# kumar-shridhar/PyTorch-BayesianCNN

Hardware: AMD Instinct MI355X
Metric: MC-forward samples/sec, BayesianAlexNet CIFAR-10 bs=512 num_ens=10 (higher is better)
Workload: dtype f32; 1 GPU; BayesianAlexNet 3x32x32 -> 10, layer_type=bbb, softplus, bs=512, num_ens=10, forward only; global_batch=512, num_ens_total=10, parallelism=single, launch=hipGraph replay, 2 lane(s) x 4 steps per launch

## Files before the change

### pytorch-bayesiancnn_amd/csrc/pconv_args.h

```cpp
#pragma once
#include <stdint.h>

struct PConvArgs {
    const float* x;
    const float* w;
    const float* w2;
    const float* bias;
    const float* bias2;
    float* y;
    float* y_mu;
    float* y_var;
    const float* eps_ext;
    int64_t x_ds, w_ds, b_ds, y_ds;
    int32_t B, Cin, H, W, Cout, kh, kw, sh, sw, ph, pw, dh, dw, Ho, Wo;
    int32_t K, Kp, khkw, act, sample;
    int32_t Mtiles, nbt, Ntiles, G, per_xcd;
    uint32_t k0, k1, call0, stream_id;
    int32_t wtap;
    uint32_t x_inv;
    const uint32_t* call_dev;
    int32_t unit_div, unit_off, x_mod, b_off;
    int32_t ksplit;
    int32_t* tickets;
    float* part;
    int32_t px_run;
    int64_t x_ps, y_ps;
    int32_t pool;
    int32_t x_div, x_off;
    int32_t y_f32;
    int32_t vh0, vh1, vw0, vw1;
    int32_t y_c8;
    int32_t up_h, up_w, tstep_h, tstep_w;
};
```

### pytorch-bayesiancnn_amd/csrc/pconv_body.cuh

```cuda
#pragma once
#include <hip/hip_runtime.h>
#include <stdint.h>

#include "bbb_common.cuh"
#include "pconv_args.h"

namespace pconv {

typedef float f32x16 __attribute__((ext_vector_type(16)));
typedef float f32x4 __attribute__((ext_vector_type(4)));

constexpr int kThreads = 256;
constexpr int BN = 64;
constexpr int BK = 32;
constexpr int LDW = BN + 1;
constexpr int KCH = 256;
constexpr int TPC = KCH / BK;

constexpr int kPlain = 0, kSplit = 1, kSeq = 2, kPool = 3;

__device__ __forceinline__ float agpr_read(float a) {
    float v;
    asm volatile("v_accvgpr_read_b32 %0, %1" : "=v"(v) : "a"(a));
    return v;
}
__device__ __forceinline__ void agpr_write(float& a, float v) { asm volatile("v_accvgpr_write_b32 %0, %1" : "=a"(a) : "v"(v)); }
template <int BM, bool LRT, bool ILV, int MODE = kPlain, bool TR = false>
__device__ __forceinline__ void pconv_item(const PConvArgs& p, const int64_t item, const int ks = 0) {
    constexpr bool SPLIT = MODE == kSplit;
    constexpr bool SEQ = MODE == kSeq;
    constexpr bool POOL = MODE == kPool;
    static_assert(!POOL || !LRT || BM == 64, "the pooled LRT form: 64-image tiles (one accumulator pair per wave)");
    static_assert(!TR || (MODE == kPlain && !LRT), "the transposed item: plain BBB form only");
    constexpr int LDX = BM + 4;
    constexpr int NT = (BM >= 128) ? 2 : 1;
    constexpr int MT = (BM == 256) ? 2 : 1;
    constexpr int WSETS = LRT ? 2 : 1;
    constexpr int XL = BM / 4;
    constexpr int XRPP = kThreads / XL;
    constexpr int XPASS = BK / XRPP;

    __shared__ __attribute__((aligned(16))) float Xs[1][BK * LDX];
    __shared__ float Ws[1][WSETS][BK * LDW];
    __shared__ int32_t kt_w[2][KCH];
    __shared__ int32_t kt_x[2][KCH];
    __shared__ float sbias[POOL ? BN : 1];
    __shared__ float sbias2[(POOL && LRT) ? BN : 1];

    int g, j;
    if (p.x_ds == 0 || (p.x_div > 1 && p.x_off == 0 && p.G % (p.x_div * p.Ntiles) == 0)) {
        const int gs = p.x_div > 1 ? p.x_div * p.Ntiles : p.G;
        const int64_t per_step = (int64_t)p.Mtiles * gs;
        const int step = (int)(item / per_step);
        const int64_t r = item - (int64_t)step * per_step;
        j = (int)(r / gs);
        g = step * gs + (int)(r - (int64_t)j * gs);
    } else {
        g = (int)(item / p.Mtiles);
        j = (int)(item - (int64_t)g * p.Mtiles);
    }
    const int e = g / p.Ntiles;
    const int ue = p.unit_off + e;
    const int ew = p.unit_div > 1 ? ue / p.unit_div : e;
    const int ex = p.x_div > 1 ? (e + p.x_off) / p.x_div : (p.x_mod > 0 ? ue % p.x_mod : e);
    const int n0 = (g - e * p.Ntiles) * BN;
    const int pix = j / p.nbt;
    const int b0 = (j - pix * p.nbt) * BM;
    const int Wq = POOL ? p.Wo / 2 : p.Wo;
    const int oh0 = pix / Wq, ow0 = pix - oh0 * Wq;
    int ihb, iwb, r_lo, q_lo, nq, nrq, Keff, ntiles;
    float inv_nrq, inv_nq;
    const float inv_cin = 1.0f / (float)p.Cin;
    auto tr_axis = [](int base, int d, int up, int step, int k, int n, int& lo, int& cnt) {
        lo = 0; cnt = 0;
        int first = -1;
        for (int r = 0; r < step && r < k; ++r)
            if ((base + r * d) % up == 0) { first = r; break; }
        if (first < 0) return;
        const int t0 = base + first * d, sd = step * d;
        const int r0 = first + (t0 < 0 ? (-t0 + sd - 1) / sd : 0) * step;
        const int lim = (n - 1) * up - base;
        if (lim < 0) return;
        int r1 = lim / d;
        r1 = r1 < k - 1 ? r1 : k - 1;
        if (r1 < r0) return;
        lo = r0; cnt = (r1 - r0) / step + 1;
    };
    auto set_pixel = [&](int oh, int ow) {
        if constexpr (POOL) {
            oh = __builtin_amdgcn_readfirstlane(oh);
            ow = __builtin_amdgcn_readfirstlane(ow);
        }
        if constexpr (TR) {
            ihb = oh - p.ph;
            iwb = ow - p.pw;
            int nr;
            tr_axis(ihb, p.dh, p.up_h, p.tstep_h, p.kh, p.H, r_lo, nr);
            tr_axis(iwb, p.dw, p.up_w, p.tstep_w, p.kw, p.W, q_lo, nq);
            nrq = nr * nq;
            Keff = p.Cin * nrq;
            ntiles = (Keff + BK - 1) / BK;
            inv_nrq = nrq > 0 ? 1.0f / (float)nrq : 0.0f;
            inv_nq = nq > 0 ? 1.0f / (float)nq : 0.0f;
            return;
        }
        ihb = oh * p.sh - p.ph;
        iwb = ow * p.sw - p.pw;
        r_lo = ihb < 0 ? (-ihb + p.dh - 1) / p.dh : 0;
        q_lo = iwb < 0 ? (-iwb + p.dw - 1) / p.dw : 0;
        int r_hi = (p.H - 1 - ihb) >= 0 ? (p.H - 1 - ihb) / p.dh + 1 : 0;
        int q_hi = (p.W - 1 - iwb) >= 0 ? (p.W - 1 - iwb) / p.dw + 1 : 0;
        r_hi = r_hi < p.kh ? r_hi : p.kh;
        q_hi = q_hi < p.kw ? q_hi : p.kw;
        const int nr = r_hi > r_lo ? r_hi - r_lo : 0;
        nq = q_hi > q_lo ? q_hi - q_lo : 0;
        nrq = nr * nq;
        Keff = p.Cin * nrq;
        ntiles = (Keff + BK - 1) / BK;
        inv_nrq = nrq > 0 ? 1.0f / (float)nrq : 0.0f;
        inv_nq = nq > 0 ? 1.0f / (float)nq : 0.0f;
    };
    set_pixel(POOL ? 2 * oh0 : oh0, POOL ? 2 * ow0 : ow0);

    const int tid = threadIdx.x;
    const int lane = tid & 63;
    const int wave = __builtin_amdgcn_readfirstlane(tid >> 6);
    const int wn = (BM >= 128) ? 0 : (wave >> 1) * 32;
    const int wm = (BM >= 128) ? wave * 32 * MT : (wave & 1) * 32;

    constexpr uint32_t kOOB = 0xFFFFFFF0u;
    constexpr uint32_t kWInv = 0x7FFFFFF0u;
    const uint32_t kXInv = p.x_inv;
    const int64_t w_elems = (int64_t)p.Cout * p.Kp;
    const int64_t x_elems = (int64_t)p.Cin * p.H * p.W * p.B;
    const __amdgpu_buffer_rsrc_t xrs = __builtin_amdgcn_make_buffer_rsrc(
        const_cast<float*>(p.x + (int64_t)ex * p.x_ds), 0, (int)(x_elems * 4), 0x00020000);
    const __amdgpu_buffer_rsrc_t wrs = __builtin_amdgcn_make_buffer_rsrc(
        const_cast<float*>(p.w + (int64_t)ew * p.w_ds), 0, (int)(w_elems * 4), 0x00020000);
    const __amdgpu_buffer_rsrc_t w2rs = __builtin_amdgcn_make_buffer_rsrc(
        const_cast<float*>(LRT ? p.w2 + (int64_t)ew * p.w_ds : p.w), 0, (int)(w_elems * 4), 0x00020000);

    const int wkl = tid & 31, wnl = tid >> 5;
    const int xb4 = (tid % XL) * 4, xkr = tid / XL;
    const uint32_t xcol = (uint32_t)(b0 + xb4) * 4u;
    uint32_t wrow[8];
#pragma unroll
    for (int ps = 0; ps < 8; ++ps) wrow[ps] = (uint32_t)(n0 + wnl + ps * 8) * (uint32_t)p.Kp * 4u;

    float wregA[WSETS][8];
    f32x4 xregA[XPASS];
// ... 4 lines not shown
        if (k < Keff) {
            int ci, rq;
            if (p.wtap) {
                rq = (int)((float)k * inv_cin);
                ci = k - rq * p.Cin;
                if (ci < 0) { --rq; ci += p.Cin; } else if (ci >= p.Cin) { ++rq; ci -= p.Cin; }
            } else {
                ci = (int)((float)k * inv_nrq);
                rq = k - ci * nrq;
                if (rq < 0) { --ci; rq += nrq; } else if (rq >= nrq) { ++ci; rq -= nrq; }
            }
            int rr = (int)((float)rq * inv_nq);
            int qq = rq - rr * nq;
            if (qq < 0) { --rr; qq += nq; } else if (qq >= nq) { ++rr; qq -= nq; }
            if constexpr (TR) {
                const int r = r_lo + rr * p.tstep_h, q = q_lo + qq * p.tstep_w;
                wo = (uint32_t)(ci * p.khkw + r * p.kw + q) * 4u;
                xo = (uint32_t)((ci * p.H + (ihb + r * p.dh) / p.up_h) * p.W + (iwb + q * p.dw) / p.up_w) * (uint32_t)p.B * 4u;
            } else {
                const int r = r_lo + rr, q = q_lo + qq;
                wo = (p.wtap ? (uint32_t)((r * p.kw + q) * p.Cin + ci) : (uint32_t)(ci * p.khkw + r * p.kw + q)) * 4u;
                xo = (uint32_t)((ci * p.H + ihb + r * p.dh) * p.W + iwb + q * p.dw) * (uint32_t)p.B * 4u;
            }
        }
        kt_w[chunk & 1][tid] = (int32_t)wo;
        kt_x[chunk & 1][tid] = (int32_t)xo;
    };

    constexpr int NLOADS = 8 + XPASS;
    uint32_t loff[NLOADS];
    auto load_addr = [&](int tile) {
        const int buf = (tile / TPC) & 1;
        const int kb = (tile % TPC) * BK;
        const uint32_t wob = (uint32_t)kt_w[buf][kb + wkl];
#pragma unroll
        for (int ps = 0; ps < 8; ++ps) loff[ps] = wrow[ps] + wob;
#pragma unroll
        for (int ps = 0; ps < XPASS; ++ps) loff[8 + ps] = (uint32_t)kt_x[buf][kb + xkr + ps * XRPP] + xcol;
    };
    auto load_one = [&](int i, float (&wreg)[WSETS][8], f32x4 (&xreg)[XPASS]) {
        if (i < XPASS) {
            xreg[i] = __builtin_bit_cast(f32x4, __builtin_amdgcn_raw_buffer_load_b128(xrs, loff[8 + i], 0, 0));
        } else {
            const int ps = i - XPASS;
            wreg[0][ps] = __builtin_bit_cast(float, __builtin_amdgcn_raw_buffer_load_b32(wrs, loff[ps], 0, 0));
            if (LRT) wreg[WSETS - 1][ps] = __builtin_bit_cast(float, __builtin_amdgcn_raw_buffer_load_b32(w2rs, loff[ps], 0, 0));
        }
    };
    auto load_tile = [&](int tile, float (&wreg)[WSETS][8], f32x4 (&xreg)[XPASS]) {
        load_addr(tile);
#pragma unroll
        for (int i = 0; i < NLOADS; ++i) load_one(i, wreg, xreg);
    };

    auto store_tile = [&](int, float (&wreg)[WSETS][8], f32x4 (&xreg)[XPASS]) {
        constexpr int buf = 0;
#pragma unroll
        for (int s = 0; s < WSETS; ++s)
#pragma unroll
            for (int ps = 0; ps < 8; ++ps) Ws[buf][s][wkl * LDW + wnl + ps * 8] = wreg[s][ps];
#pragma unroll
        for (int ps = 0; ps < XPASS; ++ps)
            *reinterpret_cast<f32x4*>(&Xs[buf][(xkr + ps * XRPP) * LDX + xb4]) = xreg[ps];
    };

    f32x16 acc[NT][MT];
    f32x16 accv[NT][MT];
    float tot[(SEQ || POOL) ? NT : 1][(SEQ || POOL) ? MT : 1][16];
    float totv[(SEQ && LRT) ? NT : 1][(SEQ && LRT) ? MT : 1][16];
#pragma unroll
    for (int t = 0; t < NT; ++t)
#pragma unroll
        for (int u = 0; u < MT; ++u)
#pragma unroll
            for (int r = 0; r < 16; ++r) {
                acc[t][u][r] = 0.0f; accv[t][u][r] = 0.0f;
                if constexpr (SEQ) { agpr_write(tot[t][u][r], 0.0f); if constexpr (LRT) agpr_write(totv[t][u][r], 0.0f); }
                if constexpr (POOL) agpr_write(tot[t][u][r], -__builtin_inff());
            }

    const int lrow = lane & 31, lk = lane >> 5;

    constexpr int PD = (BM >= 128) ? 2 : 4;
    auto mma_tile = [&](bool more) {
        float ra[PD + 1][NT], ra2[PD + 1][NT], rb[PD + 1][MT];
        auto fetch = [&](int kk, int slot) {
            const int krow = kk * 2 + lk;
#pragma unroll
            for (int mt = 0; mt < MT; ++mt) rb[slot][mt] = Xs[0][krow * LDX + wm + mt * 32 + lrow];
#pragma unroll
            for (int nt = 0; nt < NT; ++nt) {
                ra[slot][nt] = Ws[0][0][krow * LDW + wn + nt * 32 + lrow];
                if (LRT) ra2[slot][nt] = Ws[0][WSETS - 1][krow * LDW + wn + nt * 32 + lrow];
            }
        };
#pragma unroll
        for (int i = 0; i < PD; ++i) fetch(i, i);
#pragma unroll
        for (int kk = 0; kk < BK / 2; ++kk) {
            if (ILV && kk < NLOADS) {
                if (more) load_one(kk, wregA, xregA);
                __builtin_amdgcn_sched_barrier(0);
            }
            if (kk + PD < BK / 2) fetch(kk + PD, (kk + PD) % (PD + 1));
            const int s = kk % (PD + 1);
#pragma unroll
            for (int nt = 0; nt < NT; ++nt) {
#pragma unroll
                for (int mt = 0; mt < MT; ++mt)
                    acc[nt][mt] = __builtin_amdgcn_mfma_f32_32x32x2f32(ra[s][nt], rb[s][mt], acc[nt][mt], 0, 0, 0);
                if (LRT) {
#pragma unroll
                    for (int mt = 0; mt < MT; ++mt)
                        accv[nt][mt] = __builtin_amdgcn_mfma_f32_32x32x2f32(ra2[s][nt], rb[s][mt] * rb[s][mt], accv[nt][mt], 0, 0, 0);
                }
            }
            if (!ILV) __builtin_amdgcn_sched_barrier(0);
        }
    };

    if constexpr (POOL) {
        const __amdgpu_buffer_rsrc_t brs0 = __builtin_amdgcn_make_buffer_rsrc(
            const_cast<float*>(p.bias ? p.bias + (int64_t)ew * p.b_ds : p.w), 0, p.bias ? p.Cout * 4 : 0, 0x00020000);
        if (tid < BN) sbias[tid] = __builtin_bit_cast(float, __builtin_amdgcn_raw_buffer_load_b32(brs0, (uint32_t)(n0 + tid) * 4u, 0, 0));
        if constexpr (LRT) {
            const __amdgpu_buffer_rsrc_t brs2 = __builtin_amdgcn_make_buffer_rsrc(
                const_cast<float*>(p.bias2 ? p.bias2 + (int64_t)ew * p.b_ds : p.w), 0, p.bias2 ? p.Cout * 4 : 0, 0x00020000);
            if (tid < BN) sbias2[tid] = __builtin_bit_cast(float, __builtin_amdgcn_raw_buffer_load_b32(brs2, (uint32_t)(n0 + tid) * 4u, 0, 0));
        }
        __syncthreads();
    }
#pragma clang loop unroll(disable)
    for (int wp = 0; wp < (POOL ? 4 : 1); ++wp) {
    if (POOL && wp > 0) set_pixel(2 * oh0 + (wp >> 1), 2 * ow0 + (wp & 1));
    int t0 = 0, t1 = ntiles;
    if constexpr (SPLIT) {
        t0 = (int)((int64_t)ks * ntiles / p.ksplit);
        t1 = (int)((int64_t)(ks + 1) * ntiles / p.ksplit);
    }
    if (t1 > t0) {
        const int c0 = t0 / TPC;
        fill_chunk(c0);
        __syncthreads();
        load_tile(t0, wregA, xregA);
        if ((c0 + 1) * KCH < Keff) fill_chunk(c0 + 1);
        store_tile(0, wregA, xregA);
        __syncthreads();
        const int nranges = SEQ ? p.ksplit : 1;
        int t = t0;
#pragma clang loop unroll(disable)
        for (int sr = 0; sr < nranges; ++sr) {
            const int tr1 = SEQ ? (int)((int64_t)(sr + 1) * ntiles / p.ksplit) : t1;
#pragma clang loop unroll(disable)
            for (; t < tr1; ++t) {
                const bool more = (t + 1) < t1;
                if (more) {
                    if (ILV) load_addr(t + 1);
                    else     load_tile(t + 1, wregA, xregA);
                }
                if ((t % TPC) == 1 && t / TPC >= c0 + 1 && (t / TPC + 1) * KCH < Keff) fill_chunk(t / TPC + 1);
                mma_tile(more);
                __syncthreads();
                if (more) store_tile(0, wregA, xregA);
                __syncthreads();
            }
            if constexpr (SEQ) {
                if (sr + 1 < nranges) {
#pragma unroll
                    for (int nt = 0; nt < NT; ++nt)
#pragma unroll
                        for (int mt = 0; mt < MT; ++mt)
#pragma unroll
                            for (int r = 0; r < 16; ++r) {
                                agpr_write(tot[nt][mt][r], agpr_read(tot[nt][mt][r]) + acc[nt][mt][r]);
                                acc[nt][mt][r] = 0.0f;
                                if constexpr (LRT) {
                                    agpr_write(totv[nt][mt][r], agpr_read(totv[nt][mt][r]) + accv[nt][mt][r]);
                                    accv[nt][mt][r] = 0.0f;
                                }
                            }
                }
            }
        }
        if constexpr (SEQ) {
#pragma unroll
            for (int nt = 0; nt < NT; ++nt)
#pragma unroll
                for (int mt = 0; mt < MT; ++mt)
#pragma unroll
                    for (int r = 0; r < 16; ++r) {
                        acc[nt][mt][r] = agpr_read(tot[nt][mt][r]) + acc[nt][mt][r];
                        if constexpr (LRT) accv[nt][mt][r] = agpr_read(totv[nt][mt][r]) + accv[nt][mt][r];
                    }
        }
    }
    if constexpr (POOL && !LRT) {
#pragma unroll
        for (int nt = 0; nt < NT; ++nt)
#pragma unroll
            for (int r = 0; r < 16; ++r) {
                const float bn = sbias[wn + nt * 32 + (r & 3) + 8 * (r >> 2) + 4 * lk];
#pragma unroll
                for (int mt = 0; mt < MT; ++mt) {
                    const float v = bbb::apply_act(acc[nt][mt][r] + bn, p.act);
                    agpr_write(tot[nt][mt][r], fmaxf(agpr_read(tot[nt][mt][r]), v));
                    acc[nt][mt][r] = 0.0f;
                }
            }
    }
    if constexpr (POOL && LRT) {
        const int pixc = (2 * oh0 + (wp >> 1)) * p.Wo + 2 * ow0 + (wp & 1);
        const int HoWoC = p.Ho * p.Wo;
#pragma unroll
        for (int mt = 0; mt < MT; ++mt) {
            const int b = b0 + wm + mt * 32 + lrow;
            const int bglob = b + p.b_off + (p.unit_div > 1 ? (ue % p.unit_div) * p.B : 0);
#pragma unroll
            for (int nt = 0; nt < NT; ++nt)
#pragma unroll
                for (int r = 0; r < 16; ++r) {
                    const int nl = wn + nt * 32 + (r & 3) + 8 * (r >> 2) + 4 * lk;
                    const int n = n0 + nl;
                    float v = acc[nt][mt][r] + sbias[nl];
                    const float var = 1e-16f + (accv[nt][mt][r] + sbias2[nl]);
                    if (p.sample) {
                        float z;
                        if (p.eps_ext) {
                            const bool in = (b < p.B) & (n < p.Cout);
                            z = in ? p.eps_ext[(int64_t)e * ((int64_t)p.Cout * HoWoC * p.B) + ((int64_t)n * HoWoC + pixc) * p.B + b] : 0.0f;
                        } else {
                            const uint64_t idx = (uint64_t)(((int64_t)bglob * p.Cout + n) * HoWoC + pixc);
                            float z4[4];
                            bbb::normal4(idx >> 2, p.stream_id, p.call0 + (p.call_dev ? *p.call_dev : 0u) + (uint32_t)ew, p.k0, p.k1, z4);
                            const int c = (int)(idx & 3);
                            z = c == 0 ? z4[0] : c == 1 ? z4[1] : c == 2 ? z4[2] : z4[3];
                        }
                        v = v + __builtin_amdgcn_sqrtf(var) * z;
                    }
                    v = bbb::apply_act(v, p.act);
                    agpr_write(tot[nt][mt][r], fmaxf(agpr_read(tot[nt][mt][r]), v));
                    acc[nt][mt][r] = 0.0f;
                    accv[nt][mt][r] = 0.0f;
                    __builtin_amdgcn_sched_barrier(0);
                }
// ... 197 lines not shown
```

### pytorch-bayesiancnn_amd/csrc/pconv_dgrad.hip

```cpp
#include <hip/hip_runtime.h>
#include <stdint.h>

#include "../../include/bbb_hip.h"
#include "bbb_common.cuh"
#include "pconv_args.h"
#include "pconv_body.cuh"

namespace {

using namespace pconv;

template <int BM, bool ILV>
__global__ __launch_bounds__(kThreads) void pconv_dgrad_kernel(const PConvArgs p) {
    const int bid = blockIdx.x;
    const int xcd = bid & 7;
    const int64_t item = (int64_t)xcd * p.per_xcd + (bid >> 3);
    const int64_t item_end = (int64_t)(xcd + 1) * p.per_xcd;
    if (item >= item_end || item >= (int64_t)p.G * p.Mtiles) return;
    pconv_item<BM, false, ILV, kPlain, true>(p, item);
}

int gcd(int a, int b) {
    while (b != 0) { const int t = a % b; a = b; b = t; }
    return a;
}

}

extern "C" int bbb_conv2d_chwn_dgrad(const bbb_conv_desc_t* d, const float* g_pre, const float* w_flipped, float* dx, int up_h,
                                     int up_w, int out_h, int out_w, void* stream) {
    if (d == nullptr) return BBB_EINVAL;
    if (d->batch <= 0 || d->cin <= 0 || d->h <= 0 || d->w <= 0 || d->cout <= 0 || d->kh <= 0 || d->kw <= 0 || d->pad_h < 0 ||
        d->pad_w < 0 || d->dil_h <= 0 || d->dil_w <= 0 || d->draws <= 0 || up_h <= 0 || up_w <= 0 || out_h <= 0 || out_w <= 0)
        return BBB_EINVAL;
    if (d->stride_h != 1 || d->stride_w != 1) return BBB_EINVAL;
    if (up_h == 1 && up_w == 1) return BBB_EINVAL;
    if (d->act != 0 || d->pool != 0 || d->w_tap_major != 0 || d->w_row_pitch != 0 || d->unit_div != 0 || d->unit_off != 0 ||
        d->x_unit_mod != 0 || d->x_unit_div != 0 || d->x_unit_off != 0 || d->b_offset != 0)
        return BBB_EINVAL;
    if (d->x_draw_stride < 0 || d->w_draw_stride < 0) return BBB_EINVAL;
    if (d->batch % 4 != 0) return BBB_ESHAPE;
    const int fph = d->dil_h * (d->kh - 1) - d->pad_h, fpw = d->dil_w * (d->kw - 1) - d->pad_w;
    if (fph < 0 || fpw < 0) return BBB_ESHAPE;
    const int64_t nh = (int64_t)out_h + 2 * fph - (int64_t)d->dil_h * (d->kh - 1) - 1;
    const int64_t nw = (int64_t)out_w + 2 * fpw - (int64_t)d->dil_w * (d->kw - 1) - 1;
    if (nh < 0 || nw < 0 || nh / up_h + 1 != d->h || nw / up_w + 1 != d->w) return BBB_ESHAPE;
    const int64_t g_bytes = (int64_t)d->cin * d->h * d->w * d->batch * 4, dx_bytes = (int64_t)d->cout * out_h * out_w * d->batch * 4;
    if ((int64_t)d->cin * d->h * d->w > 0x7fffffffLL || (int64_t)d->cin * d->kh * d->kw > 0x7fffffffLL) return BBB_ESHAPE;
    if (g_bytes > 0xFFFE0000LL || dx_bytes > 0xFFFE0000LL || ((int64_t)d->cout + 64) * d->cin * d->kh * d->kw * 4 > 0x3FFFFFFFLL ||
        (int64_t)d->batch * 4 > 0x0FFFFFFFLL)
        return BBB_ESHAPE;
    PConvArgs a = {};
    a.x_inv = (0xFFFFFFF0u - ((uint32_t)d->batch + 512u) * 4u) & ~15u;
    if (g_bytes > (int64_t)a.x_inv) return BBB_ESHAPE;
    if (g_pre == nullptr || w_flipped == nullptr || dx == nullptr) return BBB_EINVAL;
    if ((((uintptr_t)g_pre | (uintptr_t)dx) & 15u) != 0 || (((uintptr_t)w_flipped) & 3u) != 0) return BBB_EALIGN;
    a.x = g_pre; a.w = w_flipped; a.y = dx;
    a.B = d->batch; a.Cin = d->cin; a.H = d->h; a.W = d->w; a.Cout = d->cout; a.kh = d->kh; a.kw = d->kw;
    a.sh = 1; a.sw = 1; a.ph = d->pad_h; a.pw = d->pad_w; a.dh = d->dil_h; a.dw = d->dil_w;
    a.Ho = out_h; a.Wo = out_w; a.K = d->cin * d->kh * d->kw; a.Kp = a.K; a.khkw = d->kh * d->kw;
    a.x_ds = d->x_draw_stride; a.w_ds = d->w_draw_stride;
    a.y_ds = (int64_t)d->cout * out_h * out_w * d->batch;
    a.up_h = up_h; a.up_w = up_w;
    a.tstep_h = up_h / gcd(up_h, d->dil_h); a.tstep_w = up_w / gcd(up_w, d->dil_w);
    a.Ntiles = (a.Cout + BN - 1) / BN;
    a.G = a.Ntiles * d->draws;
    const int64_t pixels = (int64_t)out_h * out_w;
    const int64_t nb128 = pixels * ((a.B + 127) / 128) * a.G;
    int bm = nb128 < 768 ? 64 : 128;
    if (bm == 128 && (a.B + 127) / 128 * 128 * 4 >= a.B * 5 && (a.B + 63) / 64 * 64 < (a.B + 127) / 128 * 128) bm = 64;
    a.nbt = (a.B + bm - 1) / bm;
    const int64_t mt = pixels * a.nbt;
    if (mt > 0x7fffffffLL) return BBB_ESHAPE;
    a.Mtiles = (int)mt;
    const int64_t items = (int64_t)a.G * mt;
    const int64_t per = (items + 7) / 8;
    if (8 * per > 0x7fffffffLL) return BBB_ESHAPE;
    a.per_xcd = (int32_t)per;
    const bool ilv = items <= 12000;
    const dim3 grid((unsigned)(8 * per)), block(kThreads);
    hipStream_t st = (hipStream_t)stream;
    if (bm == 128) {
        if (ilv) hipLaunchKernelGGL((pconv_dgrad_kernel<128, true>), grid, block, 0, st, a);
        else     hipLaunchKernelGGL((pconv_dgrad_kernel<128, false>), grid, block, 0, st, a);
    } else {
        if (ilv) hipLaunchKernelGGL((pconv_dgrad_kernel<64, true>), grid, block, 0, st, a);
        else     hipLaunchKernelGGL((pconv_dgrad_kernel<64, false>), grid, block, 0, st, a);
    }
    return (int)hipGetLastError();
}
```

### pytorch-bayesiancnn_amd/csrc/pconv_gemm.hip

```cpp
#include <hip/hip_runtime.h>
#include <stdlib.h>
#include <stdint.h>

#include "../../include/bbb_hip.h"
#include "bbb_common.cuh"
#include "pconv_args.h"
#include "pconv_body.cuh"
#include "pconv_bf16x3.cuh"

namespace {

using namespace pconv;

template <int BM, bool LRT, bool ILV, bool SEQ = false>
__global__ __launch_bounds__(kThreads) void pconv_gemm_kernel(const PConvArgs p) {
    const int bid = blockIdx.x;
    const int xcd = bid & 7;
    const int64_t item = (int64_t)xcd * p.per_xcd + (bid >> 3);
    const int64_t item_end = (int64_t)(xcd + 1) * p.per_xcd;
    if (item >= item_end || item >= (int64_t)p.G * p.Mtiles) return;
    pconv_item<BM, LRT, ILV, SEQ ? kSeq : kPlain>(p, item);
}

template <bool ILV>
__global__ __launch_bounds__(kThreads) __attribute__((amdgpu_waves_per_eu(4, 4))) void pconv_gemm_pool_kernel(const PConvArgs p) {
    const int bid = blockIdx.x;
    const int xcd = bid & 7;
    const int64_t item = (int64_t)xcd * p.per_xcd + (bid >> 3);
    const int64_t item_end = (int64_t)(xcd + 1) * p.per_xcd;
    if (item >= item_end || item >= (int64_t)p.G * p.Mtiles) return;
    pconv_item<128, false, ILV, kPool>(p, item);
}

__global__ __launch_bounds__(kThreads) void pconv_gemm_pool_lrt_kernel(const PConvArgs p) {
    const int bid = blockIdx.x;
    const int xcd = bid & 7;
    const int64_t item = (int64_t)xcd * p.per_xcd + (bid >> 3);
    const int64_t item_end = (int64_t)(xcd + 1) * p.per_xcd;
    if (item >= item_end || item >= (int64_t)p.G * p.Mtiles) return;
    pconv_item<64, true, false, kPool>(p, item);
}

template <int BM, bool LRT, bool ILV>
__global__ __launch_bounds__(kThreads) void pconv_gemm_splitk_kernel(const PConvArgs p) {
    const int bid = blockIdx.x;
    const int xcd = bid & 7;
    const int64_t blk = (int64_t)xcd * p.per_xcd + (bid >> 3);
    const int64_t blk_end = (int64_t)(xcd + 1) * p.per_xcd;
    if (blk >= blk_end || blk >= (int64_t)p.G * p.Mtiles * p.ksplit) return;
    const int64_t item = blk / p.ksplit;
    pconv_item<BM, LRT, ILV, kSplit>(p, item, (int)(blk - item * p.ksplit));
}

__global__ __launch_bounds__(256) void maxpool_chwn_kernel(const float* __restrict__ x, float* __restrict__ y, int64_t total4,
                                                           int H, int W, int Ho, int Wo, int B4, int k, int s) {
    const int64_t i = (int64_t)blockIdx.x * blockDim.x + threadIdx.x;
    if (i >= total4) return;
    const int b4 = (int)(i % B4);
    int64_t t = i / B4;
    const int ow = (int)(t % Wo);
    t /= Wo;
    const int oh = (int)(t % Ho);
    const int64_t pl = t / Ho;
    const f32x4* xp = reinterpret_cast<const f32x4*>(x) + ((pl * H + (int64_t)oh * s) * W + (int64_t)ow * s) * B4 + b4;
    f32x4 m = xp[0];
    for (int a = 0; a < k; ++a)
        for (int c = 0; c < k; ++c) {
            const f32x4 v = xp[((int64_t)a * W + c) * B4];
#pragma unroll
            for (int u = 0; u < 4; ++u) m[u] = fmaxf(m[u], v[u]);
        }
    reinterpret_cast<f32x4*>(y)[i] = m;
}

__global__ __launch_bounds__(256) void pool_act_bwd_chwn_kernel(const float* __restrict__ g_out, const float* __restrict__ y,
                                                                float* __restrict__ g_pre, int64_t total4, int H, int W, int Hp,
                                                                int Wp, int B4, int k, int s, int act, int64_t out_pitch4,
                                                                const float* __restrict__ am, const float* __restrict__ av,
                                                                float* __restrict__ g_var, int64_t mom_planes,
                                                                const float* __restrict__ g2, const float* __restrict__ xc,
                                                                int64_t xc_total4) {
    const int64_t i = (int64_t)blockIdx.x * blockDim.x + threadIdx.x;
    if (i >= total4) return;
    auto incoming = [&](int64_t idx) {
        f32x4 gv = reinterpret_cast<const f32x4*>(g_out)[idx];
        if (g2 != nullptr) {
            const f32x4 b4v = reinterpret_cast<const f32x4*>(g2)[idx], x4v = reinterpret_cast<const f32x4*>(xc)[idx % xc_total4];
#pragma unroll
            for (int u = 0; u < 4; ++u) gv[u] = fmaf(2.0f * x4v[u], b4v[u], gv[u]);
        }
        return gv;
    };
    const int b4 = (int)(i % B4);
    int64_t t = i / B4;
    const int w = (int)(t % W);
    t /= W;
    const int h = (int)(t % H);
    const int64_t pl = t / H;
    const f32x4* yp = reinterpret_cast<const f32x4*>(y) + pl * H * W * B4 + b4;
    const f32x4 me = yp[((int64_t)h * W + w) * B4];
    f32x4 g = f32x4{0.f, 0.f, 0.f, 0.f};
    if (k == 0) {
        g = incoming(i);
    } else {
        const int64_t gbase = pl * Hp * Wp * B4 + b4;
        const int ph_lo = h - k + 1 > 0 ? (h - k + 1 + s - 1) / s : 0, ph_hi = h / s < Hp - 1 ? h / s : Hp - 1;
        const int pw_lo = w - k + 1 > 0 ? (w - k + 1 + s - 1) / s : 0, pw_hi = w / s < Wp - 1 ? w / s : Wp - 1;
        for (int ph = ph_lo; ph <= ph_hi; ++ph)
            for (int pw = pw_lo; pw <= pw_hi; ++pw) {
                bool first[4] = {true, true, true, true};
                const int my = (h - ph * s) * k + (w - pw * s);
                for (int a = 0; a < k; ++a)
                    for (int c = 0; c < k; ++c) {
                        const int idx = a * k + c;
                        if (idx == my) continue;
                        const f32x4 v = yp[((int64_t)(ph * s + a) * W + (pw * s + c)) * B4];
#pragma unroll
                        for (int u = 0; u < 4; ++u) first[u] = first[u] && (idx < my ? v[u] < me[u] : v[u] <= me[u]);
                    }
                const f32x4 go = incoming(gbase + ((int64_t)ph * Wp + pw) * B4);
#pragma unroll
                for (int u = 0; u < 4; ++u) g[u] += first[u] ? go[u] : 0.0f;
            }
    }
    f32x4 o;
#pragma unroll
    for (int u = 0; u < 4; ++u) {
        float d = 1.0f;
        if (act == 1) d = me[u] > 0.0f ? 1.0f : 0.0f;
        else if (act == 2) d = me[u] > 20.0f ? 1.0f : -expm1f(-me[u]);
        o[u] = g[u] * d;
    }
    const int64_t oi = out_pitch4 ? pl * out_pitch4 + (i - pl * (int64_t)H * W * B4) : i;
    reinterpret_cast<f32x4*>(g_pre)[oi] = o;
    if (am != nullptr) {
        const int64_t in_plane = i - pl * (int64_t)H * W * B4;
        const int64_t mi = (pl % mom_planes) * ((int64_t)H * W * B4) + in_plane;
        const f32x4 a4 = reinterpret_cast<const f32x4*>(am)[mi];
        const f32x4 v4 = reinterpret_cast<const f32x4*>(av)[mi];
        f32x4 gv;
#pragma unroll
        for (int u = 0; u < 4; ++u) {
            float v = me[u];
            if (act == 2 && !(v > 20.0f)) v = v + logf(-expm1f(-v));
            const float t = (act != 0 && !(me[u] > 0.0f)) ? 0.0f : v - a4[u];
            gv[u] = (o[u] * t) / (2.0f * v4[u]);
        }
        reinterpret_cast<f32x4*>(g_var)[oi] = gv;
    }
}

int fill(const bbb_conv_desc_t* d, PConvArgs& a) {
    if (d == nullptr) return BBB_EINVAL;
    if (d->batch <= 0 || d->cin <= 0 || d->h <= 0 || d->w <= 0 || d->cout <= 0 || d->kh <= 0 || d->kw <= 0 ||
        d->stride_h <= 0 || d->stride_w <= 0 || d->pad_h < 0 || d->pad_w < 0 || d->dil_h <= 0 || d->dil_w <= 0 ||
        d->draws <= 0 || d->act < 0 || d->act > 2)
        return BBB_EINVAL;
    if (d->batch % 4 != 0) return BBB_ESHAPE;
    const int ho = (d->h + 2 * d->pad_h - d->dil_h * (d->kh - 1) - 1) / d->stride_h + 1;
    const int wo = (d->w + 2 * d->pad_w - d->dil_w * (d->kw - 1) - 1) / d->stride_w + 1;
    if (ho <= 0 || wo <= 0) return BBB_ESHAPE;
    if ((int64_t)d->cin * d->h * d->w > 0x7fffffffLL || (int64_t)d->cin * d->kh * d->kw > 0x7fffffffLL) return BBB_ESHAPE;
    if ((int64_t)d->cin * d->h * d->w * d->batch * 4 > 0xFFFE0000LL || (int64_t)d->cout * ho * wo * d->batch * 4 > 0xFFFE0000LL ||
        ((int64_t)d->cout + 64) * d->cin * d->kh * d->kw * 4 > 0x3FFFFFFFLL || (int64_t)d->batch * 4 > 0x0FFFFFFFLL)
        return BBB_ESHAPE;
    a.x_inv = (0xFFFFFFF0u - ((uint32_t)d->batch + 512u) * 4u) & ~15u;
    if ((int64_t)d->cin * d->h * d->w * d->batch * 4 > (int64_t)a.x_inv) return BBB_ESHAPE;
    a.B = d->batch; a.Cin = d->cin; a.H = d->h; a.W = d->w; a.Cout = d->cout; a.kh = d->kh; a.kw = d->kw;
    a.sh = d->stride_h; a.sw = d->stride_w; a.ph = d->pad_h; a.pw = d->pad_w; a.dh = d->dil_h; a.dw = d->dil_w;
    a.Ho = ho; a.Wo = wo; a.K = d->cin * d->kh * d->kw; a.khkw = d->kh * d->kw; a.act = d->act;
    if (d->w_row_pitch < 0 || (d->w_row_pitch > 0 && d->w_row_pitch < a.K)) return BBB_EINVAL;
    a.Kp = d->w_row_pitch > 0 ? d->w_row_pitch : a.K;
    if (((int64_t)d->cout + 64) * a.Kp * 4 > 0x3FFFFFFFLL) return BBB_ESHAPE;
    a.x_ds = d->x_draw_stride; a.w_ds = d->w_draw_stride; a.b_ds = d->b_draw_stride;
    a.y_ds = (int64_t)d->cout * ho * wo * d->batch;
    if (d->unit_div < 0 || d->unit_off < 0 || d->x_unit_mod < 0 || d->b_offset < 0) return BBB_EINVAL;
    if (d->unit_div > 1 && d->unit_off >= d->unit_div) return BBB_EINVAL;
    if (d->x_unit_mod > 0 && d->x_unit_mod != d->unit_div) return BBB_EINVAL;
    if (d->x_unit_div < 0 || d->x_unit_off < 0 || (d->x_unit_div > 1 && (d->unit_div > 1 || d->x_unit_off >= d->x_unit_div)) ||
        (d->x_unit_div <= 1 && d->x_unit_off != 0))
        return BBB_EINVAL;
    a.unit_div = d->unit_div; a.unit_off = d->unit_div > 1 ? d->unit_off : 0; a.x_mod = d->x_unit_mod; a.b_off = d->b_offset;
    a.x_div = d->x_unit_div; a.x_off = d->x_unit_off;
    if (d->pool != 0 && d->pool != 1) return BBB_EINVAL;
    a.pool = d->pool;
    if (d->w_tap_major != 0 && d->w_tap_major != 1) return BBB_EINVAL;
    a.wtap = d->w_tap_major;
    if (a.pool) {
        if ((ho & 1) || (wo & 1)) return BBB_EINVAL;
        a.y_ds = (int64_t)d->cout * (ho / 2) * (wo / 2) * d->batch;
    }
    return 0;
}

#ifndef PCONV_ILV_MAX
#define PCONV_ILV_MAX 12000
#endif
#ifndef PCONV_SPLIT_MAX
#define PCONV_SPLIT_MAX 384
#endif
constexpr int64_t split_max_items(bool lrt) { return lrt ? 512 : PCONV_SPLIT_MAX; }

template <bool LRT>
int launch(PConvArgs& a, int draws, hipStream_t st) {
    a.Ntiles = (a.Cout + BN - 1) / BN;
    a.G = a.Ntiles * draws;
    const int64_t pixels = (int64_t)a.Ho * a.Wo;
    if (a.pool) {
        if (a.ksplit > 1 || a.part != nullptr) return BBB_EINVAL;
        if (LRT && (a.y_mu != nullptr || a.y_var != nullptr)) return BBB_EINVAL;
        a.nbt = (a.B + (LRT ? 63 : 127)) / (LRT ? 64 : 128);
        const int64_t mtp = (pixels / 4) * a.nbt;
        const int64_t itp = (int64_t)a.G * mtp;
        if (mtp > 0x7fffffffLL || itp > 0x7fffffffLL - 8) return BBB_ESHAPE;
        a.Mtiles = (int)mtp;
        const int64_t perp = (itp + 7) / 8;
        a.per_xcd = (int32_t)perp;
        if constexpr (LRT) hipLaunchKernelGGL(pconv_gemm_pool_lrt_kernel, dim3((unsigned)(8 * perp)), dim3(kThreads), 0, st, a);
        else               hipLaunchKernelGGL((pconv_gemm_pool_kernel<false>), dim3((unsigned)(8 * perp)), dim3(kThreads), 0, st, a);
        return (int)hipGetLastError();
    }
    const int64_t nb128 = pixels * ((a.B + 127) / 128) * a.G;
    int bm = (LRT || nb128 < 768) ? 64 : 128;
    if (bm == 128 && (a.B + 127) / 128 * 128 * 4 >= a.B * 5 && (a.B + 63) / 64 * 64 < (a.B + 127) / 128 * 128) bm = 64;
    const int64_t items64 = pixels * ((a.B + 63) / 64) * a.G;
    const bool cross = a.ksplit > 1 && a.part != nullptr && items64 <= split_max_items(LRT);
    if (cross) bm = 64;
    a.nbt = (a.B + bm - 1) / bm;
    const int64_t mt = pixels * a.nbt;
    if (mt > 0x7fffffffLL) return BBB_ESHAPE;
    a.Mtiles = (int)mt;
    const int64_t items = (int64_t)a.G * mt;
    if (cross) {
        if (items * a.ksplit > 0x7fffffffLL) return BBB_EINVAL;
        const int64_t perb = (items * a.ksplit + 7) / 8;
        a.per_xcd = (int32_t)perb;
        hipLaunchKernelGGL((pconv_gemm_splitk_kernel<64, LRT, true>), dim3((unsigned)(8 * perb)), dim3(kThreads), 0, st, a);
        return (int)hipGetLastError();
    }
    const int64_t per = (items + 7) / 8;
    const int64_t blocks = 8 * per;
    if (blocks > 0x7fffffffLL) return BBB_ESHAPE;
    a.per_xcd = (int32_t)per;
    const bool ilv = items <= PCONV_ILV_MAX;
    const dim3 grid((unsigned)blocks), block(kThreads);
    if (a.ksplit > 1) {
        if constexpr (!LRT) {
            if (bm == 128) {
                if (ilv) hipLaunchKernelGGL((pconv_gemm_kernel<128, false, true, true>), grid, block, 0, st, a);
                else     hipLaunchKernelGGL((pconv_gemm_kernel<128, false, false, true>), grid, block, 0, st, a);
                return (int)hipGetLastError();
            }
        }
        const bool ilv_seq = ilv && !LRT;
        if (ilv_seq) hipLaunchKernelGGL((pconv_gemm_kernel<64, LRT, true, true>), grid, block, 0, st, a);
        else         hipLaunchKernelGGL((pconv_gemm_kernel<64, LRT, false, true>), grid, block, 0, st, a);
        return (int)hipGetLastError();
    }
    if constexpr (!LRT) {
        if (bm == 128) {
            if (ilv) hipLaunchKernelGGL((pconv_gemm_kernel<128, false, true>), grid, block, 0, st, a);
            else     hipLaunchKernelGGL((pconv_gemm_kernel<128, false, false>), grid, block, 0, st, a);
            return (int)hipGetLastError();
        }
    }
    if (ilv) hipLaunchKernelGGL((pconv_gemm_kernel<64, LRT, true>), grid, block, 0, st, a);
    else     hipLaunchKernelGGL((pconv_gemm_kernel<64, LRT, false>), grid, block, 0, st, a);
    return (int)hipGetLastError();
}

}

namespace {
constexpr int64_t kTicketBytes = 16384;

int canonical_ksplit(const PConvArgs& a) {
    const int ntl = (a.Cout + BN - 1) / BN;
    const int64_t groups = (int64_t)a.Ho * a.Wo * ntl;
    if (groups > 16) return 1;
    const int nr = a.kh < (a.H - 1) / a.dh + 1 ? a.kh : (a.H - 1) / a.dh + 1;
    const int nq = a.kw < (a.W - 1) / a.dw + 1 ? a.kw : (a.W - 1) / a.dw + 1;
    const int tiles = (a.Cin * nr * nq + BK - 1) / BK;
    if (tiles < 16) return 1;
    const int s = tiles / 8;
    return s > 4 ? 4 : s;
}

int64_t split_scratch_bytes(const PConvArgs& a, int draws, bool lrt, int s) {
    if (s <= 1) return 0;
    const int ntl = (a.Cout + BN - 1) / BN;
    const int64_t items = (int64_t)a.Ho * a.Wo * ((a.B + 63) / 64) * ntl * draws;
    if (items > split_max_items(lrt)) return 0;
    return kTicketBytes + items * s * (lrt ? 2 : 1) * 64 * 64 * 4;
}

int split_setup(PConvArgs& a, int draws, bool lrt, int k_split, void* scratch, int64_t scratch_bytes) {
    if (k_split <= 1) return 0;
    if (k_split != canonical_ksplit(a)) return BBB_EINVAL;
    a.ksplit = k_split;
    const int64_t need = split_scratch_bytes(a, draws, lrt, k_split);
    if (need > 0 && scratch != nullptr) {
        if (scratch_bytes < need || (((uintptr_t)scratch) & 255u) != 0) return BBB_EINVAL;
        a.tickets = static_cast<int32_t*>(scratch);
        a.part = reinterpret_cast<float*>(static_cast<char*>(scratch) + kTicketBytes);
    }
    return 0;
}
}

extern "C" int64_t bbb_conv2d_chwn_splitk_scratch(const bbb_conv_desc_t* d, int lrt, int32_t* k_split) {
    PConvArgs a = {};
    if (k_split) *k_split = 1;
    if (fill(d, a) != 0) return 0;
    const int s = canonical_ksplit(a);
    if (k_split) *k_split = s;
    return split_scratch_bytes(a, d->draws, lrt != 0, s);
}

extern "C" int bbb_conv2d_chwn_splitk_fwd(const bbb_conv_desc_t* d, const float* x, const float* w, const float* bias, float* y,
                                          int k_split, void* scratch, int64_t scratch_bytes, void* stream) {
    PConvArgs a = {};
    int rc = fill(d, a);
    if (rc != 0) return rc;
    if (x == nullptr || w == nullptr || y == nullptr) return BBB_EINVAL;
    if ((((uintptr_t)x | (uintptr_t)y) & 15u) != 0 || (((uintptr_t)w | (uintptr_t)bias) & 3u) != 0) return BBB_EALIGN;
    a.x = x; a.w = w; a.bias = bias; a.y = y;
    if ((rc = split_setup(a, d->draws, false, k_split, scratch, scratch_bytes)) != 0) return rc;
    return launch<false>(a, d->draws, (hipStream_t)stream);
}

extern "C" int bbb_conv2d_chwn_fwd(const bbb_conv_desc_t* d, const float* x, const float* w, const float* bias, float* y,
                                   void* stream) {
    PConvArgs a = {};
    const int rc = fill(d, a);
    if (rc != 0) return rc;
    if (x == nullptr || w == nullptr || y == nullptr) return BBB_EINVAL;
    if ((((uintptr_t)x | (uintptr_t)y) & 15u) != 0 || (((uintptr_t)w | (uintptr_t)bias) & 3u) != 0) return BBB_EALIGN;
    a.x = x; a.w = w; a.bias = bias; a.y = y;
    return launch<false>(a, d->draws, (hipStream_t)stream);
}

extern "C" int bbb_conv2d_chwn_bf16x3_fwd(const bbb_conv_desc_t* d, const void* x, const float* w, const float* bias, void* y,
                                          uint32_t flags, void* stream) {
    PConvArgs a = {};
    const int rc = fill(d, a);
    if (rc != 0) return rc;
    if (x == nullptr || w == nullptr || y == nullptr || (flags & ~3u) != 0 || a.pool || a.wtap) return BBB_EINVAL;
    if ((((uintptr_t)x | (uintptr_t)y) & 15u) != 0 || (((uintptr_t)w | (uintptr_t)bias) & 3u) != 0) return BBB_EALIGN;
    const bool xs3 = (flags & BBB_S3_IN) != 0, ys3 = (flags & BBB_S3_OUT) != 0;
    if ((xs3 || ys3) && d->batch % 8 != 0) return BBB_ESHAPE;
    a.x = static_cast<const float*>(x); a.w = w; a.bias = bias; a.y = static_cast<float*>(y);
// ... 233 lines not shown
```

Before: 8.217 million samples/s.

## Skip padded MFMA steps in partial K tiles and reorder pooled tiles by work

Adds a KT template path that computes how many K pairs in the current tile are valid and skips LDS fetches and MFMA issues for the zero-padded remainder. It is enabled only when some output position has Cin*taps not divisible by BK. The pooled GEMM also gets a host-computed permutation of pooled pixels, sorted by K-tile count and dealt out serpentine across XCD groups, to balance load between blocks with border and interior pixels. The cost is extra template instantiations, a larger kernel argument struct (256-byte order table), and runtime branches in the MMA loop.

```diff
diff --git a/pytorch-bayesiancnn_amd/csrc/pconv_args.h b/pytorch-bayesiancnn_amd/csrc/pconv_args.h
--- a/pytorch-bayesiancnn_amd/csrc/pconv_args.h
+++ b/pytorch-bayesiancnn_amd/csrc/pconv_args.h
@@ -31,4 +31,6 @@
     int32_t vh0, vh1, vw0, vw1;
     int32_t y_c8;
     int32_t up_h, up_w, tstep_h, tstep_w;
+    int32_t pool_perm;
+    uint8_t pool_order[256];
 };
diff --git a/pytorch-bayesiancnn_amd/csrc/pconv_body.cuh b/pytorch-bayesiancnn_amd/csrc/pconv_body.cuh
--- a/pytorch-bayesiancnn_amd/csrc/pconv_body.cuh
+++ b/pytorch-bayesiancnn_amd/csrc/pconv_body.cuh
@@ -1,6 +1,8 @@
 #pragma once
 #include <hip/hip_runtime.h>
 #include <stdint.h>
+
+#include <type_traits>
 
 #include "bbb_common.cuh"
 #include "pconv_args.h"
@@ -25,7 +27,7 @@
     return v;
 }
 __device__ __forceinline__ void agpr_write(float& a, float v) { asm volatile("v_accvgpr_write_b32 %0, %1" : "=a"(a) : "v"(v)); }
-template <int BM, bool LRT, bool ILV, int MODE = kPlain, bool TR = false>
+template <int BM, bool LRT, bool ILV, int MODE = kPlain, bool TR = false, bool KT = false>
 __device__ __forceinline__ void pconv_item(const PConvArgs& p, const int64_t item, const int ks = 0) {
     constexpr bool SPLIT = MODE == kSplit;
     constexpr bool SEQ = MODE == kSeq;
@@ -64,8 +66,9 @@
     const int ew = p.unit_div > 1 ? ue / p.unit_div : e;
     const int ex = p.x_div > 1 ? (e + p.x_off) / p.x_div : (p.x_mod > 0 ? ue % p.x_mod : e);
     const int n0 = (g - e * p.Ntiles) * BN;
-    const int pix = j / p.nbt;
-    const int b0 = (j - pix * p.nbt) * BM;
+    const int pixi = j / p.nbt;
+    const int b0 = (j - pixi * p.nbt) * BM;
+    const int pix = (POOL && p.pool_perm) ? (int)p.pool_order[pixi] : pixi;
     const int Wq = POOL ? p.Wo / 2 : p.Wo;
     const int oh0 = pix / Wq, ow0 = pix - oh0 * Wq;
     int ihb, iwb, r_lo, q_lo, nq, nrq, Keff, ntiles;
@@ -236,7 +239,8 @@
     const int lrow = lane & 31, lk = lane >> 5;
 
     constexpr int PD = (BM >= 128) ? 2 : 4;
-    auto mma_tile = [&](bool more) {
+    auto mma_tile = [&](bool more, int t) {
+        const int live = KT ? __builtin_amdgcn_readfirstlane((Keff - t * BK + 1) >> 1) : BK / 2;
         float ra[PD + 1][NT], ra2[PD + 1][NT], rb[PD + 1][MT];
         auto fetch = [&](int kk, int slot) {
             const int krow = kk * 2 + lk;
@@ -249,24 +253,27 @@
             }
         };
 #pragma unroll
-        for (int i = 0; i < PD; ++i) fetch(i, i);
+        for (int i = 0; i < PD; ++i)
+            if (!KT || i < live) fetch(i, i);
 #pragma unroll
         for (int kk = 0; kk < BK / 2; ++kk) {
             if (ILV && kk < NLOADS) {
                 if (more) load_one(kk, wregA, xregA);
                 __builtin_amdgcn_sched_barrier(0);
             }
-            if (kk + PD < BK / 2) fetch(kk + PD, (kk + PD) % (PD + 1));
+            if (kk + PD < BK / 2 && (!KT || kk + PD < live)) fetch(kk + PD, (kk + PD) % (PD + 1));
             const int s = kk % (PD + 1);
-#pragma unroll
-            for (int nt = 0; nt < NT; ++nt) {
-#pragma unroll
-                for (int mt = 0; mt < MT; ++mt)
-                    acc[nt][mt] = __builtin_amdgcn_mfma_f32_32x32x2f32(ra[s][nt], rb[s][mt], acc[nt][mt], 0, 0, 0);
-                if (LRT) {
+            if (!KT || kk < live) {
+#pragma unroll
+                for (int nt = 0; nt < NT; ++nt) {
 #pragma unroll
                     for (int mt = 0; mt < MT; ++mt)
-                        accv[nt][mt] = __builtin_amdgcn_mfma_f32_32x32x2f32(ra2[s][nt], rb[s][mt] * rb[s][mt], accv[nt][mt], 0, 0, 0);
+                        acc[nt][mt] = __builtin_amdgcn_mfma_f32_32x32x2f32(ra[s][nt], rb[s][mt], acc[nt][mt], 0, 0, 0);
+                    if (LRT) {
+#pragma unroll
+                        for (int mt = 0; mt < MT; ++mt)
+                            accv[nt][mt] = __builtin_amdgcn_mfma_f32_32x32x2f32(ra2[s][nt], rb[s][mt] * rb[s][mt], accv[nt][mt], 0, 0, 0);
+                    }
                 }
             }
             if (!ILV) __builtin_amdgcn_sched_barrier(0);
@@ -313,7 +320,7 @@
                     else     load_tile(t + 1, wregA, xregA);
                 }
                 if ((t % TPC) == 1 && t / TPC >= c0 + 1 && (t / TPC + 1) * KCH < Keff) fill_chunk(t / TPC + 1);
-                mma_tile(more);
+                mma_tile(more, t);
                 __syncthreads();
                 if (more) store_tile(0, wregA, xregA);
                 __syncthreads();
diff --git a/pytorch-bayesiancnn_amd/csrc/pconv_dgrad.hip b/pytorch-bayesiancnn_amd/csrc/pconv_dgrad.hip
--- a/pytorch-bayesiancnn_amd/csrc/pconv_dgrad.hip
+++ b/pytorch-bayesiancnn_amd/csrc/pconv_dgrad.hip
@@ -10,14 +10,14 @@
 
 using namespace pconv;
 
-template <int BM, bool ILV>
+template <int BM, bool ILV, bool KT>
 __global__ __launch_bounds__(kThreads) void pconv_dgrad_kernel(const PConvArgs p) {
     const int bid = blockIdx.x;
     const int xcd = bid & 7;
     const int64_t item = (int64_t)xcd * p.per_xcd + (bid >> 3);
     const int64_t item_end = (int64_t)(xcd + 1) * p.per_xcd;
     if (item >= item_end || item >= (int64_t)p.G * p.Mtiles) return;
-    pconv_item<BM, false, ILV, kPlain, true>(p, item);
+    pconv_item<BM, false, ILV, kPlain, true, KT>(p, item);
 }
 
 int gcd(int a, int b) {
@@ -80,12 +80,17 @@
     const bool ilv = items <= 12000;
     const dim3 grid((unsigned)(8 * per)), block(kThreads);
     hipStream_t st = (hipStream_t)stream;
-    if (bm == 128) {
-        if (ilv) hipLaunchKernelGGL((pconv_dgrad_kernel<128, true>), grid, block, 0, st, a);
-        else     hipLaunchKernelGGL((pconv_dgrad_kernel<128, false>), grid, block, 0, st, a);
-    } else {
-        if (ilv) hipLaunchKernelGGL((pconv_dgrad_kernel<64, true>), grid, block, 0, st, a);
-        else     hipLaunchKernelGGL((pconv_dgrad_kernel<64, false>), grid, block, 0, st, a);
-    }
+    auto go = [&](auto kt) {
+        constexpr bool KT = decltype(kt)::value;
+        if (bm == 128) {
+            if (ilv) hipLaunchKernelGGL((pconv_dgrad_kernel<128, true, KT>), grid, block, 0, st, a);
+            else     hipLaunchKernelGGL((pconv_dgrad_kernel<128, false, KT>), grid, block, 0, st, a);
+        } else {
+            if (ilv) hipLaunchKernelGGL((pconv_dgrad_kernel<64, true, KT>), grid, block, 0, st, a);
+            else     hipLaunchKernelGGL((pconv_dgrad_kernel<64, false, KT>), grid, block, 0, st, a);
+        }
+    };
+    if (a.Cin % BK != 0) go(std::true_type{});
+    else                 go(std::false_type{});
     return (int)hipGetLastError();
 }
diff --git a/pytorch-bayesiancnn_amd/csrc/pconv_gemm.hip b/pytorch-bayesiancnn_amd/csrc/pconv_gemm.hip
--- a/pytorch-bayesiancnn_amd/csrc/pconv_gemm.hip
+++ b/pytorch-bayesiancnn_amd/csrc/pconv_gemm.hip
@@ -12,36 +12,37 @@
 
 using namespace pconv;
 
-template <int BM, bool LRT, bool ILV, bool SEQ = false>
+template <int BM, bool LRT, bool ILV, bool SEQ = false, bool KT = false>
 __global__ __launch_bounds__(kThreads) void pconv_gemm_kernel(const PConvArgs p) {
     const int bid = blockIdx.x;
     const int xcd = bid & 7;
     const int64_t item = (int64_t)xcd * p.per_xcd + (bid >> 3);
     const int64_t item_end = (int64_t)(xcd + 1) * p.per_xcd;
     if (item >= item_end || item >= (int64_t)p.G * p.Mtiles) return;
-    pconv_item<BM, LRT, ILV, SEQ ? kSeq : kPlain>(p, item);
-}
-
-template <bool ILV>
+    pconv_item<BM, LRT, ILV, SEQ ? kSeq : kPlain, false, KT>(p, item);
+}
+
+template <bool ILV, bool KT = false>
 __global__ __launch_bounds__(kThreads) __attribute__((amdgpu_waves_per_eu(4, 4))) void pconv_gemm_pool_kernel(const PConvArgs p) {
     const int bid = blockIdx.x;
     const int xcd = bid & 7;
     const int64_t item = (int64_t)xcd * p.per_xcd + (bid >> 3);
     const int64_t item_end = (int64_t)(xcd + 1) * p.per_xcd;
     if (item >= item_end || item >= (int64_t)p.G * p.Mtiles) return;
-    pconv_item<128, false, ILV, kPool>(p, item);
-}
-
+    pconv_item<128, false, ILV, kPool, false, KT>(p, item);
+}
+
+template <bool KT>
 __global__ __launch_bounds__(kThreads) void pconv_gemm_pool_lrt_kernel(const PConvArgs p) {
     const int bid = blockIdx.x;
     const int xcd = bid & 7;
     const int64_t item = (int64_t)xcd * p.per_xcd + (bid >> 3);
     const int64_t item_end = (int64_t)(xcd + 1) * p.per_xcd;
     if (item >= item_end || item >= (int64_t)p.G * p.Mtiles) return;
-    pconv_item<64, true, false, kPool>(p, item);
-}
-
-template <int BM, bool LRT, bool ILV>
+    pconv_item<64, true, false, kPool, false, KT>(p, item);
+}
+
+template <int BM, bool LRT, bool ILV, bool KT = false>
 __global__ __launch_bounds__(kThreads) void pconv_gemm_splitk_kernel(const PConvArgs p) {
     const int bid = blockIdx.x;
     const int xcd = bid & 7;
@@ -49,7 +50,7 @@
     const int64_t blk_end = (int64_t)(xcd + 1) * p.per_xcd;
     if (blk >= blk_end || blk >= (int64_t)p.G * p.Mtiles * p.ksplit) return;
     const int64_t item = blk / p.ksplit;
-    pconv_item<BM, LRT, ILV, kSplit>(p, item, (int)(blk - item * p.ksplit));
+    pconv_item<BM, LRT, ILV, kSplit, false, KT>(p, item, (int)(blk - item * p.ksplit));
 }
 
 __global__ __launch_bounds__(256) void maxpool_chwn_kernel(const float* __restrict__ x, float* __restrict__ y, int64_t total4,
@@ -201,8 +202,48 @@
 #endif
 constexpr int64_t split_max_items(bool lrt) { return lrt ? 512 : PCONV_SPLIT_MAX; }
 
-template <bool LRT>
-int launch(PConvArgs& a, int draws, hipStream_t st) {
+#ifndef PCONV_POOL_ORDER
+#define PCONV_POOL_ORDER 1
+#endif
+void pool_order(PConvArgs& a, int bm) {
+    a.pool_perm = 0;
+    const int Hq = a.Ho / 2, Wq = a.Wo / 2, P = Hq * Wq;
+    if (!PCONV_POOL_ORDER || P < 2 || P > 256) return;
+    auto taps = [](int o, int s, int pd, int d, int k, int n) {
+        int c = 0;
+        for (int r = 0; r < k; ++r) { const int t = o * s - pd + r * d; c += (t >= 0 && t < n); }
+        return c;
+    };
+    int len[256], idx[256];
+    for (int ph = 0; ph < Hq; ++ph)
+        for (int pw = 0; pw < Wq; ++pw) {
+            int t = 0;
+            for (int wp = 0; wp < 4; ++wp)
+                t += (a.Cin * taps(2 * ph + (wp >> 1), a.sh, a.ph, a.dh, a.kh, a.H) * taps(2 * pw + (wp & 1), a.sw, a.pw, a.dw, a.kw, a.W) + BK - 1) / BK;
+            len[ph * Wq + pw] = t;
+            idx[ph * Wq + pw] = ph * Wq + pw;
+        }
+    for (int i = 1; i < P; ++i) {
+        const int v = idx[i];
+        int j = i;
+        for (; j > 0 && len[idx[j - 1]] < len[v]; --j) idx[j] = idx[j - 1];
+        idx[j] = v;
+    }
+    const bool step_major = a.x_ds == 0 || (a.x_div > 1 && a.x_off == 0 && a.G % (a.x_div * a.Ntiles) == 0);
+    const int64_t sweep = step_major ? (int64_t)a.Mtiles * (a.x_div > 1 ? a.x_div * a.Ntiles : a.G) : a.Mtiles;
+    int c = 1;
+    if (sweep % a.per_xcd == 0 && sweep / a.per_xcd <= P && P % (sweep / a.per_xcd) == 0) c = (int)(sweep / a.per_xcd);
+    const int per = P / c;
+    int fill[256] = {0};
+    for (int i = 0; i < P; ++i) {
+        const int rnd = i / c, pos = i % c, grp = (rnd & 1) ? c - 1 - pos : pos;
+        a.pool_order[grp * per + fill[grp]++] = (uint8_t)idx[i];
+    }
+    a.pool_perm = 1;
+}
+
+template <bool LRT, bool KT>
+int launch_kt(PConvArgs& a, int draws, hipStream_t st) {
     a.Ntiles = (a.Cout + BN - 1) / BN;
     a.G = a.Ntiles * draws;
     const int64_t pixels = (int64_t)a.Ho * a.Wo;
@@ -216,8 +257,9 @@
         a.Mtiles = (int)mtp;
         const int64_t perp = (itp + 7) / 8;
         a.per_xcd = (int32_t)perp;
-        if constexpr (LRT) hipLaunchKernelGGL(pconv_gemm_pool_lrt_kernel, dim3((unsigned)(8 * perp)), dim3(kThreads), 0, st, a);
-        else               hipLaunchKernelGGL((pconv_gemm_pool_kernel<false>), dim3((unsigned)(8 * perp)), dim3(kThreads), 0, st, a);
+        pool_order(a, LRT ? 64 : 128);
+        if constexpr (LRT) hipLaunchKernelGGL((pconv_gemm_pool_lrt_kernel<KT>), dim3((unsigned)(8 * perp)), dim3(kThreads), 0, st, a);
+        else               hipLaunchKernelGGL((pconv_gemm_pool_kernel<false, KT>), dim3((unsigned)(8 * perp)), dim3(kThreads), 0, st, a);
         return (int)hipGetLastError();
     }
     const int64_t nb128 = pixels * ((a.B + 127) / 128) * a.G;
@@ -235,7 +277,7 @@
         if (items * a.ksplit > 0x7fffffffLL) return BBB_EINVAL;
         const int64_t perb = (items * a.ksplit + 7) / 8;
         a.per_xcd = (int32_t)perb;
-        hipLaunchKernelGGL((pconv_gemm_splitk_kernel<64, LRT, true>), dim3((unsigned)(8 * perb)), dim3(kThreads), 0, st, a);
+        hipLaunchKernelGGL((pconv_gemm_splitk_kernel<64, LRT, true, KT>), dim3((unsigned)(8 * perb)), dim3(kThreads), 0, st, a);
         return (int)hipGetLastError();
     }
     const int64_t per = (items + 7) / 8;
@@ -247,26 +289,50 @@
     if (a.ksplit > 1) {
         if constexpr (!LRT) {
             if (bm == 128) {
-                if (ilv) hipLaunchKernelGGL((pconv_gemm_kernel<128, false, true, true>), grid, block, 0, st, a);
-                else     hipLaunchKernelGGL((pconv_gemm_kernel<128, false, false, true>), grid, block, 0, st, a);
+                if (ilv) hipLaunchKernelGGL((pconv_gemm_kernel<128, false, true, true, KT>), grid, block, 0, st, a);
+                else     hipLaunchKernelGGL((pconv_gemm_kernel<128, false, false, true, KT>), grid, block, 0, st, a);
                 return (int)hipGetLastError();
             }
         }
         const bool ilv_seq = ilv && !LRT;
-        if (ilv_seq) hipLaunchKernelGGL((pconv_gemm_kernel<64, LRT, true, true>), grid, block, 0, st, a);
-        else         hipLaunchKernelGGL((pconv_gemm_kernel<64, LRT, false, true>), grid, block, 0, st, a);
+        if (ilv_seq) hipLaunchKernelGGL((pconv_gemm_kernel<64, LRT, true, true, KT>), grid, block, 0, st, a);
+        else         hipLaunchKernelGGL((pconv_gemm_kernel<64, LRT, false, true, KT>), grid, block, 0, st, a);
         return (int)hipGetLastError();
     }
     if constexpr (!LRT) {
         if (bm == 128) {
-            if (ilv) hipLaunchKernelGGL((pconv_gemm_kernel<128, false, true>), grid, block, 0, st, a);
-            else     hipLaunchKernelGGL((pconv_gemm_kernel<128, false, false>), grid, block, 0, st, a);
+            if (ilv) hipLaunchKernelGGL((pconv_gemm_kernel<128, false, true, false, KT>), grid, block, 0, st, a);
+            else     hipLaunchKernelGGL((pconv_gemm_kernel<128, false, false, false, KT>), grid, block, 0, st, a);
             return (int)hipGetLastError();
         }
     }
-    if (ilv) hipLaunchKernelGGL((pconv_gemm_kernel<64, LRT, true>), grid, block, 0, st, a);
-    else     hipLaunchKernelGGL((pconv_gemm_kernel<64, LRT, false>), grid, block, 0, st, a);
+    if (ilv) hipLaunchKernelGGL((pconv_gemm_kernel<64, LRT, true, false, KT>), grid, block, 0, st, a);
+    else     hipLaunchKernelGGL((pconv_gemm_kernel<64, LRT, false, false, KT>), grid, block, 0, st, a);
     return (int)hipGetLastError();
+}
+
+bool has_partial_tile(const PConvArgs& a) {
+    if (a.Cin % BK == 0) return false;
+    auto counts = [](int no, int s, int pd, int d, int k, int n, bool* seen) {
+        for (int o = 0; o < no; ++o) {
+            int c = 0;
+            for (int r = 0; r < k; ++r) { const int t = o * s - pd + r * d; c += (t >= 0 && t < n); }
+            seen[c < 64 ? c : 64] = true;
+        }
+    };
+    bool nr[65] = {false}, nq[65] = {false};
+    if (a.kh > 64 || a.kw > 64 || (int64_t)a.Ho * a.kh + (int64_t)a.Wo * a.kw > (1 << 16)) return true;
+    counts(a.Ho, a.sh, a.ph, a.dh, a.kh, a.H, nr);
+    counts(a.Wo, a.sw, a.pw, a.dw, a.kw, a.W, nq);
+    for (int i = 1; i <= a.kh; ++i)
+        for (int j = 1; j <= a.kw; ++j)
+            if (nr[i] && nq[j] && ((int64_t)a.Cin * i * j) % BK != 0) return true;
+    return false;
+}
+
+template <bool LRT>
+int launch(PConvArgs& a, int draws, hipStream_t st) {
+    return has_partial_tile(a) ? launch_kt<LRT, true>(a, draws, st) : launch_kt<LRT, false>(a, draws, st);
 }
 
 }
```

Result: no change. 8.229 million samples/s (median of 3 runs) (+0.2%).
